# sdu-hpcl/BGSA

Measured on AMD Instinct MI355X. Metric: GCUPS (cell updates/sec) all-pairs Myers 150bp, higher is better.
Workload: dtype u32

## Files before the change

bgsa_amd/__init__.py:

```python
from __future__ import annotations

import ctypes
import os
import subprocess
from pathlib import Path

import numpy as np

HERE = Path(__file__).resolve().parent
LIB_PATH = Path(os.environ["BGSA_HIP_LIB"]) if os.environ.get("BGSA_HIP_LIB") else HERE / "libbgsa_hip.so"
LIB_AB_PATH = HERE / "libbgsa_hip_ab.so"
INCLUDE = HERE.parent / "include" / "bgsa_hip.h"

ALGO_MYERS, ALGO_BANDED, ALGO_BITPAL = 0, 1, 2
DISTANCE_BEYOND = -2
V_NUM = 64

_lib = None


class Params(ctypes.Structure):
    _fields_ = [("algo", ctypes.c_int), ("alignment", ctypes.c_int), ("match", ctypes.c_int),
                ("mismatch", ctypes.c_int), ("gap", ctypes.c_int), ("k", ctypes.c_int)]

# ... 148 lines not shown
    L.bgsa_hip_bucket_release.argtypes = [vp]
    u64p = ctypes.POINTER(ctypes.c_uint64)
    L.bgsa_hip_seam_stats.argtypes = [u64p, u64p, u64p]
    L.bgsa_hip_row_cache_stats.argtypes = [u64p, u64p]
    L.bgsa_hip_event_create.argtypes = [ctypes.POINTER(vp)]
    L.bgsa_hip_event_destroy.argtypes = [vp]
    L.bgsa_hip_event_record.argtypes = [vp, vp]
    L.bgsa_hip_event_synchronize.argtypes = [vp]
    L.bgsa_hip_event_elapsed_ms.argtypes = [vp, vp, ctypes.POINTER(ctypes.c_float)]
    L.bgsa_hip_stream_wait_event.argtypes = [vp, vp]
    L.bgsa_hip_query_stream.argtypes = [i32, vp, i32, i32, vp, i32]
    L.bgsa_hip_myers_band_stream.argtypes = [vp, i32, i32, vp, i32]
    L.bgsa_hip_myers_band_half.argtypes = [i32, i32]
    L.bgsa_hip_myers_band_stats.argtypes = [vp, i32]
    if hasattr(L, "bgsa_hip_myers_band_groups"):
        L.bgsa_hip_myers_band_groups.argtypes = [i32, i64, i32, i32, i32]
    if hasattr(L, "bgsa_hip_myers_band_rescue"):
        L.bgsa_hip_myers_band_rescue.argtypes = [i32, i32, i32, i64]
        L.bgsa_hip_myers_band_rescue_half.argtypes = [i32]
        L.bgsa_hip_myers_band_rescue_stats.argtypes = [vp, i32]
    if hasattr(L, "bgsa_hip_myers_prefix_depths"):
        L.bgsa_hip_myers_prefix_depths.argtypes = [i32, i64, i32, i32, i32, i32, ip, i32]
        L.bgsa_hip_myers_band_segments.argtypes = [vp, i32, i32, ip, i32, vp, i32, ip]
    L.bgsa_hip_kernel_name.argtypes = [i32, i32]
    L.bgsa_hip_kernel_name.restype = ctypes.c_char_p
    L.bgsa_hip_malloc.argtypes = [ctypes.POINTER(vp), sz]
    L.bgsa_hip_free.argtypes = [vp]
    L.bgsa_hip_malloc_host.argtypes = [ctypes.POINTER(vp), sz]
    L.bgsa_hip_free_host.argtypes = [vp]
    L.bgsa_hip_memcpy_h2d.argtypes = [vp, vp, sz, vp]
    L.bgsa_hip_memcpy_d2h.argtypes = [vp, vp, sz, vp]
    L.bgsa_hip_memset.argtypes = [vp, i32, sz, vp]
    L.bgsa_hip_stream_synchronize.argtypes = [vp]
    L.bgsa_hip_stream_create.argtypes = [ctypes.POINTER(vp)]
    L.bgsa_hip_stream_destroy.argtypes = [vp]
    L.bgsa_hip_set_device.argtypes = [i32]
    L.hip_handle_reads.argtypes = [vp, vp, i32, i64, i64]
    L.hip_handle_reads.restype = None
    L.hip_cal_align_score.argtypes = [vp, vp, vp, i32, i32, i32, i32, i32, i32, i32, i32, vp]
    L.hip_cal_align_score.restype = None
    L.align_hip.argtypes = [vp, vp, i32, i32, i32, i32, i32, vp, vp]
    L.align_hip.restype = None
    L.init_mapping_table.restype = None
    L.malloc_mem.argtypes = [ctypes.c_uint64]
    L.malloc_mem.restype = vp
    L.free_mem.argtypes = [vp]
# ... 766 lines not shown
```

bgsa_amd/csrc/bgsa_common.h:

```cpp
#pragma once

#include <hip/hip_runtime.h>
#include <stdint.h>
#include <stdlib.h>
#include <stdio.h>

#include <type_traits>

#include "../../include/bgsa_hip.h"

namespace bgsa {

constexpr int kLanes = HIP_V_NUM;
constexpr int kChars = BGSA_CHAR_NUM;
constexpr int kWavesPerBlock = 4;
constexpr int kMaxWords = 32;

void set_error(const char *what, hipError_t e, const char *file, int line);
void set_error_text(const char *text);
int refuse(const char *who, int rc, const char *why);

#define BGSA_HIP_TRY(expr)                                              \
    do {                                                                \
        hipError_t e_ = (expr);                                         \
// ... 43 lines not shown
    template <typename F>
    static int dispatch(int nw, const char *family, F &&f)
    {
        int rc = BGSA_HIP_EUNSUPPORTED;
        if (((N == nw ? (rc = f(std::integral_constant<int, N>{}), true) : false) || ...)) return rc;
        char msg[128];
        snprintf(msg, sizeof msg, "%s: no kernel of %d words in this build", family, nw);
        set_error_text(msg);
        return BGSA_HIP_EUNSUPPORTED;
    }
    template <int M>
    constexpr Widths<N..., M> with() const { return {}; }
};
template <typename A, typename B> struct JoinWidths;
template <int... A, int... B> struct JoinWidths<Widths<A...>, Widths<B...>> { using type = Widths<A..., B...>; };
template <typename A, typename B> using Join = typename JoinWidths<A, B>::type;

int launch_myers(const ScoreArgs &a, int semi_global = 0);
int launch_myers_place_lens(const ScoreArgs &a);
const char *myers_kernel_name(int word_num, int semi_global = 0);
int myers_band_groups(int word_num, int64_t read_count, int ref_len, int read_len, int mixed_lengths);
int myers_prefix_depths(int word_num, int64_t read_count, int ref_len, int read_len, int n_queries, int mixed_lengths, int *depths);
int myers_band_rescue(int ref_len, int read_len, int n_queries, int64_t read_count);

constexpr int kCodeEnd = 5, kCodeRefill = 6;
inline int stream_windows(int ref_len) { return ref_len / 7 + 1; }
inline size_t stream_stride(int ref_len) { return static_cast<size_t>(stream_windows(ref_len) + 1) * 8; }
__host__ __device__ inline unsigned long long plain_stream_window(const char *row, int ref_len, int i)
{
    const int n_windows = ref_len / 7 + 1;
    unsigned long long win = 0;
    for (int j = 0; j < 8; j++) {
        unsigned code = kCodeEnd;
        if (i < n_windows) {
            const int pos = 7 * i + j;
            if (j == 7) code = (i < n_windows - 1) ? kCodeRefill : kCodeEnd;
            else if (pos < ref_len) {
                code = static_cast<unsigned char>(row[pos]);
                if (code > 4) code = 0;
            }
        }
        win |= static_cast<unsigned long long>(code) << (8 * j);
    }
    return win;
}
int launch_pack_queries(const char *d_content, int ref_len, int ref_start, int ref_end,
// ... 444 lines not shown
```

bgsa_amd/csrc/capi.hip:

```cpp
#include <stdlib.h>
#include <string.h>

#include <algorithm>
#include <atomic>
#include <chrono>
#include <map>
#include <memory>
#include <mutex>
#include <string>
#include <thread>
#include <utility>
#include <vector>

#include "bgsa_common.h"
#include "myers_band.h"

namespace bgsa {

static thread_local std::string g_last_error;

void set_error(const char *what, hipError_t e, const char *file, int line)
{
    char buf[512];
    snprintf(buf, sizeof buf, "%s failed: %s (%s:%d)", what, hipGetErrorString(e), file, line);
// ... 563 lines not shown
    for (int j = 0; j < n && j < cap; j++) depths[j] = d[j];
    return n;
}

int bgsa_hip_myers_band_segments(const char *mapped_row, int ref_len, int read_len, const int *depths, int n_depths,
                                 unsigned char *dst, int cap, int *offsets)
{
    if (!mapped_row || ref_len <= 0 || read_len <= 0 || !depths || n_depths < 1 || n_depths > kPrefixMaxDepths) return 0;
    BandSchedule s;
    if (!band_schedule(ref_len, read_len, band_half(ref_len, read_len), (read_len + 31) / 32, &s)) return 0;
    PrefixPlan p;
    p.n = n_depths;
    for (int j = 0; j < n_depths; j++) p.depth[j] = depths[j];
    if (!prefix_plan_layout(ref_len, (read_len + 31) / 32, s, &p)) return 0;
    const int n = p.off[p.n + 1];
    if (offsets)
        for (int j = 0; j <= p.n + 1; j++) offsets[j] = p.off[j];
    if (dst && cap >= n)
        for (int i = 0; i < n / 8; i++) {
            int seg = 0;
            while (seg < p.n && p.off[seg + 1] <= 8 * i) seg++;
            for (int j = 0; j < 8; j++) dst[8 * i + j] = kCodeEnd;
            band_rows_layout(s, seg ? p.depth[seg - 1] : 0, seg < p.n ? p.depth[seg] : ref_len, seg == p.n, mapped_row, dst + 8 * i,
                             8 * i - p.off[seg], 8);
        }
    return n;
}

int bgsa_hip_myers_band_stream(const char *mapped_row, int ref_len, int read_len, unsigned char *dst, int cap)
{
    if (!mapped_row || ref_len <= 0 || read_len <= 0) return BGSA_HIP_EINVAL;
    BandSchedule s;
    if (!band_schedule(ref_len, read_len, band_half(ref_len, read_len), (read_len + 31) / 32, &s)) return 0;
    const int n = band_stream_layout(ref_len, s, mapped_row, nullptr);
    if (dst && cap >= n)
        for (int i = 0; 8 * i < n; i++) {
            memset(dst + 8 * i, kCodeEnd, 8);
            band_stream_layout(ref_len, s, mapped_row, dst + 8 * i, 8 * i, 8);
        }
    return n;
}

int bgsa_hip_myers_band_stats(unsigned long long *out, int clear)
{
    if (!out) return BGSA_HIP_EINVAL;
    out[0] = out[1] = 0;
// ... 1184 lines not shown
```

bgsa_amd/csrc/myers_band.h:

```cpp
#pragma once

#include <stdlib.h>

#include "bgsa_common.h"

namespace bgsa {

constexpr int kBandMaxWords = 8;
constexpr int kBandMinWords = 3;
constexpr int kBandMaxSwitches = 2 * kBandMaxWords;
constexpr int kCodeSetWin = 7;
constexpr int kBandBadCode = 0xff;

struct BandSchedule {
    int n = 0;
    int row[kBandMaxSwitches] = {};
    int win[kBandMaxSwitches] = {};
};

__host__ __device__ inline int band_window_index(int nw, int a, int b) { return a * nw - a * (a - 1) / 2 + (b - a); }

inline int band_default_half(int len) { return (9 * len + 192) / 32; }

inline int band_rescue_half(int len) { return band_default_half(len) - 3; }

inline int band_half(int m, int n, bool rescue = false)
{
    static const int knob = [] {
        const char *e = getenv("BGSA_MYERS_BAND");
        return e ? atoi(e) : -1;
    }();
    if (knob >= 0) return knob;
    return rescue ? band_rescue_half(m > n ? m : n) : band_default_half(m > n ? m : n);
}

inline bool band_schedule(int m, int n, int h, int nw, BandSchedule *s)
{
    s->n = 0;
    const int B = 2 * h + 1, delta = n - m;
    if (h <= 0 || m <= 0 || n <= 0 || abs(delta) > B || nw < kBandMinWords || nw > kBandMaxWords || (n + 31) / 32 != nw)
        return false;
    const int dlo = -((B - delta) / 2), dhi = (delta + B) / 2;
    long long words = 0;
// ... 1 lines not shown
    for (int i = 1; i <= m; i++) {
        const int jlo = i + dlo < 1 ? 1 : i + dlo, jhi = i + dhi > n ? n : i + dhi;
        const int a = (jlo - 1) / 32, b = (jhi - 1) / 32;
        words += b - a + 1;
        if (a != pa || b != pb) {
            if (s->n == kBandMaxSwitches) {
                s->n = 0;
                return false;
            }
            s->row[s->n] = i - 1;
            s->win[s->n] = band_window_index(nw, a, b);
            s->n++;
            pa = a;
            pb = b;
        }
    }
    if (5 * words > 4ll * m * nw) {
        s->n = 0;
        return false;
    }
    return true;
}

inline size_t band_stream_stride(int ref_len) { return stream_stride(ref_len + 3 * kBandMaxSwitches); }

__host__ __device__ inline int band_rows_layout(const BandSchedule &s, int r0, int r1, bool spare, const char *row, unsigned char *dst,
                                                int first = 0, int count = 0x7fffffff)
{
    int pos = 0, sw = 0;
    auto in = [&]() { return dst && pos >= first && pos - first < count; };
    auto put = [&](int c) {
        if (in()) dst[pos - first] = static_cast<unsigned char>(c);
        pos++;
    };
    auto refill = [&]() {
        put(kCodeRefill);
        while (pos & 7) put(kCodeEnd);
    };
    while (sw + 1 < s.n && s.row[sw + 1] <= r0) sw++;
    for (int r = r0; r < r1; r++) {
        if (dst && pos - first >= count) return pos;
        if (sw < s.n && (s.row[sw] == r || r == r0)) {
            if ((pos & 7) >= 6) refill();
            put(kCodeSetWin);
            put(s.win[sw]);
            sw++;
// ... 122 lines not shown
```

bgsa_amd/csrc/myers_global.hip:

```cpp
#include <stdlib.h>
#include <string.h>

#include <algorithm>

#include "bgsa_common.h"
#include "myers_band.h"

namespace bgsa {

template <int NW, int G, bool SEMI = false>
__device__ __forceinline__ void myers_row(uint32_t (&vp)[G * NW], uint32_t (&vn)[G * NW],
                                          const uint32_t (&eq)[G * NW], int last_word = 0, int last_bit = 0,
                                          int *delta = nullptr)
{
#pragma unroll
  for (int gi = 0; gi < G; gi++) {
    uint32_t hp_prev = 0, hn_prev = 0;
    unsigned carry = 0;
#pragma unroll
    for (int ww = 0; ww < NW; ww++) {
        const int w = gi * NW + ww;
        const uint32_t pv = vp[w], mv = vn[w], e = eq[w];
        const uint32_t pm = e | mv;
        unsigned cout;
// ... 106 lines not shown
    asm volatile("v_mbcnt_lo_u32_b32 %0, -1, 0\n\tv_mbcnt_hi_u32_b32 %0, -1, %0" : "=v"(l));
    return l;
}
constexpr int band_kernel_waves(int nw, int g, bool dyn, bool share)
{
    if (!share) return 1;
    if (g == 2) return nw == 3 ? 8 : (nw == 4 ? (dyn ? 6 : 7) : 5);
    return nw <= 5 ? 8 : (nw == 6 ? (dyn ? 7 : 8) : (nw == 7 ? (dyn ? 6 : 7) : (dyn ? 5 : 6)));
}
template <int NW, int G, bool DYN = false, bool BAND = false, bool LENS = false, bool SHARE = false, bool RESCUE = false>
__global__ __launch_bounds__(256) __attribute__((amdgpu_waves_per_eu(band_kernel_waves(NW, G, DYN, SHARE)))) void myers_global_asm_kernel(
    const unsigned char *__restrict__ streams, const uint32_t *__restrict__ peq,
    int16_t *__restrict__ out, int ref_len, int read_len, long long ld, int n_groups, int word_num,
    int n_queries, int q_tile, int stream_stride_bytes, unsigned *__restrict__ fault_word,
    unsigned *__restrict__ task_counter, int band_limit = 0, unsigned long long *__restrict__ band_launch = nullptr,
    const int32_t *__restrict__ read_lens = nullptr, unsigned long long prefix_segments = 0,
    const PrefixEntry *__restrict__ order = nullptr)
{
    static_assert(!BAND || (NW >= kBandMinWords && NW <= kBandMaxWords && (G == 1 || (G == 2 && NW <= kBandPairMaxWords))),
                  "band: 3..8 words, one subject group per wave — or two up to 5 words");
    static_assert(!(LENS && BAND), "the certified band is derived from one (m, n): a length-aware launch runs full rows");
    static_assert(!SHARE || BAND, "prefix sharing: the band kernels only");
    static_assert(!RESCUE || (BAND && G == 2), "rescue: the two-group band kernels only");
    constexpr bool kLenPerQuery = LENS && NW > 8;
    const int lane = threadIdx.x & (kLanes - 1);
    const unsigned wave_groups = (static_cast<unsigned>(n_groups) + G - 1) / G;
    const unsigned n_tasks = wave_groups * ((static_cast<unsigned>(n_queries) + q_tile - 1) / q_tile);
    unsigned task = 0, task_issued = 0;
    if constexpr (DYN) {
        task = first_wave_task();
        if (task >= n_tasks) return;
    }
    int band_on = 1, unreported = 0;
    [[maybe_unused]] auto reporting_lane = [&]() {
        if constexpr (RESCUE) {
            return lane_now() == 0;
        } else
            return lane == 0;
    };
    do {
        int group0, tile;
        if constexpr (DYN) {
            group0 = static_cast<int>((task % wave_groups) * G);
            tile = static_cast<int>(task / wave_groups);
        } else {
            group0 = __builtin_amdgcn_readfirstlane((blockIdx.x * kWavesPerBlock + (threadIdx.x >> 6)) * G);
// ... 27 lines not shown
        for (int k = q0; k < q1; k++) {
            if constexpr (DYN) {
                if (k == q1 - 1) task_issued = issue_wave_task(task_counter);
            }
            int q = k, seg = 0;
            if constexpr (SHARE) {
                const int2 e = *reinterpret_cast<const int2 *>(order + k);
                q = __builtin_amdgcn_readfirstlane(e.x);
                seg = __builtin_amdgcn_readfirstlane(e.y >> 16);
            }
            uint32_t st[2 * G * NW];
#pragma unroll
            for (int w = 0; w < G * NW; w++) {
                st[2 * w] = ~0u;
                st[2 * w + 1] = 0u;
            }
            const unsigned long long s =
                reinterpret_cast<unsigned long long>(streams) + static_cast<unsigned long long>(q) * stream_stride_bytes;
            if constexpr (BAND) {
                const int n_live = G == 1 ? 1 : (group0 + 1 < n_groups ? 2 : 1);
                const int tried = band_on * n_live;
                int band = band_on, score[G];
                const int n_depths = SHARE ? static_cast<int>(prefix_segments >> 56) : 0;
                const bool sharing = SHARE && band_on;
                [[maybe_unused]] auto wave_slots = [&]() {
                    if constexpr (RESCUE) {
                        return prefix_slots + __builtin_amdgcn_readfirstlane((threadIdx.x >> 6) * G) * kLanes + lane_now();
                    } else
                        return prefix_slots + ((threadIdx.x >> 6) * G) * kLanes + lane;
                };
                if (!sharing) seg = 0;
                if (SHARE && seg) {
                    const uint4 *const slots = wave_slots();
#pragma unroll
                    for (int gi = 0; gi < G; gi++) {
                        const uint4 v = slots[((seg - 1) * kWavesPerBlock * G + gi) * kLanes];
                        st[2 * gi * NW] = v.x;
                        st[2 * gi * NW + 1] = v.y;
                        st[2 * gi * NW + 2] = v.z;
                        st[2 * gi * NW + 3] = v.w;
                    }
                }
                for (;;) {
                    for (; seg <= n_depths; seg++) {
                        const int at = SHARE ? static_cast<int>((prefix_segments >> (8 * seg)) & 0xffu) * 8 : 0;
                        const int left = myers_band_rows_asm<NW, G>(st, P, uniform_u64(s + static_cast<unsigned>(at)),
                                                                    __builtin_amdgcn_readfirstlane((stream_stride_bytes - at) / 8 - 2),
                                                                    __builtin_amdgcn_readfirstlane(band));
                        note_stream_fault(fault_word, left);
                        if (SHARE && sharing && band && seg < n_depths) {
                            uint4 *const slots = wave_slots();
#pragma unroll
                            for (int gi = 0; gi < G; gi++)
                                slots[(seg * kWavesPerBlock * G + gi) * kLanes] =
                                    make_uint4(st[2 * gi * NW], st[2 * gi * NW + 1], st[2 * gi * NW + 2], st[2 * gi * NW + 3]);
                        }
                    }
#pragma unroll
                    for (int gi = 0; gi < G; gi++) {
                        score[gi] = ref_len;
#pragma unroll
                        for (int w = 0; w < NW; w++) {
                            const int rem = read_len - 32 * w;
                            const uint32_t m = rem >= 32 ? ~0u : (rem <= 0 ? 0u : ((1u << rem) - 1u));
                            score[gi] += __popc(st[2 * (gi * NW + w)] & m) - __popc(st[2 * (gi * NW + w) + 1] & m);
                        }
                    }
                    if (!band) break;
                    int n_over = 0;
#pragma unroll
                    for (int gi = 0; gi < G; gi++)
                        if (gi < n_live && __builtin_amdgcn_ballot_w64(score[gi] > band_limit) != 0) n_over++;
                    if (n_over == 0) break;
                    if constexpr (G == 1) n_over = 1;
                    if constexpr (RESCUE) {
                        const unsigned c0 = __popcll(__builtin_amdgcn_ballot_w64(score[0] > band_limit)),
                                       c1 = n_live > 1 ? __popcll(__builtin_amdgcn_ballot_w64(score[1] > band_limit)) : 0u;
                        unsigned forced = (c0 > kRescueMaxLanes ? 1u : 0u) + (c1 > kRescueMaxLanes ? 1u : 0u);
                        if (forced == 0) {
                            unsigned *const words = reinterpret_cast<unsigned *>(band_launch) - 16;
                            unsigned long long claim = 0;
                            if (reporting_lane()) claim = atomicAdd(rescue_claimed(words), static_cast<unsigned long long>(c0 + c1));
                            const unsigned base = __builtin_amdgcn_readfirstlane(static_cast<unsigned>(claim)),
                                           base_hi = __builtin_amdgcn_readfirstlane(static_cast<unsigned>(claim >> 32));
                            const unsigned capacity = __builtin_amdgcn_readfirstlane(*rescue_capacity(words));
                            const unsigned room = (base_hi == 0 && base < capacity) ? capacity - base : 0u;
                            const bool fits = c0 + c1 <= room;
                            RescueEntry *const mine = rescue_pool(words) + base;
                            const unsigned column = lane_now() + static_cast<unsigned>(group0) * kLanes;
#pragma unroll
                            for (int gi = 0; gi < G; gi++) {
                                const bool up = gi < n_live && score[gi] > band_limit;
                                const unsigned long long over = __builtin_amdgcn_ballot_w64(up);
                                const unsigned at = (gi ? c0 : 0u) + __builtin_amdgcn_mbcnt_hi(static_cast<unsigned>(over >> 32),
                                                                                              __builtin_amdgcn_mbcnt_lo(static_cast<unsigned>(over), 0u));
                                if (up && at < room)
                                    mine[at] = fits ? RescueEntry{q, static_cast<int>(column + gi * kLanes)} : RescueEntry{-1, -1};
                            }
                            if (fits) break;
                            forced = static_cast<unsigned>(n_over);
                        }
                        if (reporting_lane()) atomicAdd(&band_launch[3], static_cast<unsigned long long>(forced));
                    }
                    band = 0;
                    seg = 0;
                    unsigned long long r = static_cast<unsigned long long>(n_over),
                                       b = static_cast<unsigned long long>(unreported) + n_live;
                    if (reporting_lane()) {
                        r += atomicAdd(&band_launch[0], r);
                        b += atomicAdd(&band_launch[1], b);
                    }
                    r = uniform_u64(r);
                    b = uniform_u64(b);
                    unreported = -n_live;
                    if (b >= 64 && 8 * r > b) band_on = 0;
#pragma unroll
                    for (int w = 0; w < G * NW; w++) {
                        st[2 * w] = ~0u;
                        st[2 * w + 1] = 0u;
                    }
                }
                unreported += tried;
#pragma unroll
                for (int gi = 0; gi < G; gi++)
                    if (gi < n_live && !(RESCUE && band && score[gi] > band_limit))
                        dst[static_cast<size_t>(q) * ld + gi * kLanes] = static_cast<int16_t>(-score[gi]);
            } else {
                int left;
                if constexpr (NW <= kPairMaxWords)
                    left = myers_pair_rows_asm<NW, G>(st, P, uniform_u64(s), __builtin_amdgcn_readfirstlane(stream_stride_bytes / 8 - 2));
                else
                    left = myers_rows_asm<NW, G>(st, P, uniform_u64(s), __builtin_amdgcn_readfirstlane(stream_stride_bytes / 8 - 2));
                note_stream_fault(fault_word, left);
#pragma unroll
                for (int gi = 0; gi < G; gi++) {
                    int score = ref_len;
                    int n_cols = read_len;
                    if constexpr (kLenPerQuery) {
                        const unsigned lane_e = lane_now();
                        n_cols = group0 + gi < n_groups ? lane_read_len(read_lens, static_cast<size_t>(group0 + gi) * kLanes + lane_e, read_len) : 0;
                    }
                    else if constexpr (LENS)
                        n_cols = own_len[gi];
                    if constexpr (LENS) asm volatile("" : "+v"(n_cols));
#pragma unroll
                    for (int w = 0; w < NW; w++) {
                        const int rem = n_cols - 32 * w;
                        const uint32_t m = rem >= 32 ? ~0u : (rem <= 0 ? 0u : ((1u << rem) - 1u));
// ... 483 lines not shown
long long rescue_entries_for(int ref_len, int read_len, int nq, int64_t read_count)
{
    if (read_len < kRescueMinLen || read_len > kRescueMaxLen || nq <= 0 || read_count < 2 * kLanes || read_count > 0x7fffffffll) return 0;
    const long long pool = static_cast<long long>(rescue_pool_bytes(read_len, nq) / sizeof(RescueEntry));
    long long entries = rescue_pool_entries(read_len, nq);
    if (rescue_pool_knob() >= 0 && rescue_pool_knob() < entries) entries = rescue_pool_knob();
    if (rescue_knob() >= 0) return rescue_knob() ? entries : 0;
    if (!kRescueDefault || nq < kRescueMinQueries || read_count < kBandPairMinReads || !band_rescue_lengths(ref_len, read_len)) return 0;
    return 2e-3 * nq * static_cast<double>(read_count) <= static_cast<double>(pool / 2) ? entries : 0;
}
int band_half_for(int ref_len, int read_len, int nw, int groups, int nq, int64_t read_count, BandSchedule *sched, long long *entries)
{
    *entries = groups == 2 && nw <= kBandPairMaxWords ? rescue_entries_for(ref_len, read_len, nq, read_count) : 0;
    if (*entries > 0) {
        const int h = band_half(ref_len, read_len, true);
        if (band_schedule(ref_len, read_len, h, nw, sched)) return h;
        *entries = 0;
    }
    const int h = band_half(ref_len, read_len);
    band_schedule(ref_len, read_len, h, nw, sched);
    return h;
}

template <int NW>
__global__ __launch_bounds__(256) void myers_band_rescue_kernel(unsigned *__restrict__ words, const char *__restrict__ content,
                                                                const uint32_t *__restrict__ peq, int16_t *__restrict__ out,
                                                                int ref_len, int read_len, long long ld, int word_num, int ref_start,
                                                                int n_queries)
{
    const unsigned long long claimed = *rescue_claimed(words), capacity = *rescue_capacity(words);
    const unsigned long long count = claimed < capacity ? claimed : capacity;
    const RescueEntry *pool = rescue_pool(words);
    const unsigned lane = threadIdx.x & (kLanes - 1);
    const unsigned long long n_waves = static_cast<unsigned long long>(gridDim.x) * kWavesPerBlock;
    unsigned rescued = 0;
    for (unsigned long long chunk = static_cast<unsigned long long>(blockIdx.x) * kWavesPerBlock + (threadIdx.x >> 6);
         chunk * kLanes < count; chunk += n_waves) {
        const unsigned long long at = chunk * kLanes + lane;
        RescueEntry e = pool[at < count ? at : count - 1];
        const bool live = at < count && e.q >= 0 && e.q < n_queries && e.subject >= 0 && e.subject < ld;
        if (!live) e = RescueEntry{0, 0};
        const uint32_t *g = peq + (static_cast<size_t>(e.subject / kLanes) * kChars * word_num) * kLanes + e.subject % kLanes;
        uint32_t P[kChars][NW], pv[NW], mv[NW];
#pragma unroll
        for (int c = 0; c < kChars; c++)
#pragma unroll
// ... 41 lines not shown
    const bool lens = a.d_read_lens != nullptr;
    const int64_t n_waves = (a.n_groups() + G - 1) / G;
    const TaskPlan plan = plan_tasks(nq, n_waves, static_cast<long long>(a.ref_len) * NW * G, NW >= 30 ? 8 : 32, kCounter,
                                     NW >= 30 ? long_query_tile() : query_tile_max(), lens);
    if (lens && kCounter && !plan.dynamic) {
        set_error_text("myers: too many tasks for one length-aware launch (split the query window)");
        return BGSA_HIP_EUNSUPPORTED;
    }
    note_query_tile(plan.q_tile);
    AsmKernel on_grid = nullptr, on_counter = nullptr;
    if constexpr (!kBandPair) {
        on_grid = myers_global_asm_kernel<NW, G, false>;
        if constexpr (kCounter) on_counter = myers_global_asm_kernel<NW, G, true>;
        if (lens) {
            if constexpr (kCounter) on_grid = nullptr, on_counter = myers_global_asm_kernel<NW, G, true, false, true>;
            else on_grid = myers_global_asm_kernel<NW, G, false, false, true>;
        }
    }
    BandSchedule sched;
    PrefixPlan prefix;
    int h = 0;
    bool band = false;
    long long rescue = 0;
    if constexpr ((G == 1 || kBandPair) && NW >= kBandMinWords && NW <= kBandMaxWords) {
        if (!lens) h = band_half_for(a.ref_len, a.read_len, NW, G, nq, a.read_count, &sched, &rescue);
        band = !lens && sched.n > 0;
        if (band) {
            on_grid = myers_global_asm_kernel<NW, G, false, true>;
            on_counter = myers_global_asm_kernel<NW, G, true, true>;
            prefix_select(a.ref_len, NW, sched, nq, plan.q_tile, a.read_count, &prefix);
            if (prefix.n) {
                on_grid = myers_global_asm_kernel<NW, G, false, true, false, true>;
                on_counter = myers_global_asm_kernel<NW, G, true, true, false, true>;
            }
            if constexpr (kBandPair) {
                if (rescue > 0) {
                    on_grid = prefix.n ? myers_global_asm_kernel<NW, G, false, true, false, true, true>
                                       : myers_global_asm_kernel<NW, G, false, true, false, false, true>;
                    on_counter = prefix.n ? myers_global_asm_kernel<NW, G, true, true, false, true, true>
                                          : myers_global_asm_kernel<NW, G, true, true, false, false, true>;
                }
            }
        }
    }
    if (kBandPair && !band) {
        set_error_text("myers: two subject groups per wave selected for a launch without the certified band");
        return BGSA_HIP_EUNSUPPORTED;
    }
    const unsigned lds = (plan.dynamic ? myers_lds_pad() : 0u) + static_cast<unsigned>(prefix_lds_bytes(prefix, G));
    const int stride = static_cast<int>(prefix.n  ? static_cast<size_t>(prefix.off[prefix.n + 1])
                                        : band    ? band_stream_stride(a.ref_len)
                                        : kPairs  ? pair_stream_stride(a.ref_len)
                                                  : stream_stride(a.ref_len));
    unsigned *words = task_counter_in(a.d_workspace, static_cast<size_t>(stride) * nq);
    LaunchGrid lg;
    if (int rc = plan_grid(plan, n_waves, nq, words,
                           [&] { return on_counter ? persistent_blocks_for(on_counter, lds) : persistent_blocks(); }, "myers", &lg))
        return rc;
    if (prefix.n)
        if (int rc = launch_prefix_order(a.d_content, a.ref_len, a.ref_start, a.ref_end, plan.q_tile, prefix, words, a.stream))
            return rc;
    if (int rc = prefix.n ? launch_pack_band_segments(a.d_content, a.ref_len, sched, prefix, a.ref_start, a.ref_end, a.d_workspace, a.stream, words,
                                                       static_cast<unsigned>(rescue))
                 : band   ? launch_pack_band(a.d_content, a.ref_len, sched, a.ref_start, a.ref_end, a.d_workspace, a.stream, words,
                                             static_cast<unsigned>(rescue))
                 : kPairs ? launch_pack_query_pairs(a.d_content, a.ref_len, a.ref_start, a.ref_end, a.d_workspace, a.stream, lg.counter)
                          : launch_pack_queries(a.d_content, a.ref_len, a.ref_start, a.ref_end, a.d_workspace, a.stream, lg.counter))
        return rc;
    unsigned *fault = nullptr;
    if (int rc = stream_guard(a.d_workspace, stride, kPairs ? kPairRefill : kCodeRefill, band ? kBandBadCode : kPairs ? -1 : 7, a.stream, &fault))
        return rc;
    unsigned long long *guard = band ? band_launch_words(words) : nullptr;
    const AsmKernel kernel = lg.counter ? on_counter : on_grid;
    hipLaunchKernelGGL(kernel, lg.grid, dim3(256), lds, a.stream,
                       static_cast<const unsigned char *>(a.d_workspace), a.d_peq, a.results<int16_t>(), a.ref_len, a.read_len,
                       static_cast<long long>(a.read_count), static_cast<int>(a.n_groups()), a.word_num, nq, plan.q_tile, stride,
                       fault, lg.counter, band ? 2 * h + 1 : 0, guard, a.d_read_lens, prefix_segments_word(prefix),
                       static_cast<const PrefixEntry *>(prefix_entries(words)));
    BGSA_HIP_TRY(hipGetLastError());
    if constexpr (kBandPair) {
        if (rescue > 0) {
            hipLaunchKernelGGL(myers_band_rescue_kernel<NW>, dim3(persistent_blocks()), dim3(256), 0, a.stream, words, a.d_content, a.d_peq,
                               a.results<int16_t>(), a.ref_len, a.read_len, static_cast<long long>(a.read_count), a.word_num,
                               a.ref_start, nq);
            BGSA_HIP_TRY(hipGetLastError());
        }
    }
    if (band) {
        hipLaunchKernelGGL(band_stats_add_kernel, dim3(1), dim3(1), 0, a.stream, static_cast<const unsigned long long *>(guard),
                           band_stats_words(fault));
        BGSA_HIP_TRY(hipGetLastError());
    }
    return BGSA_HIP_OK;
}

template <int NW, bool LENS = false>
int launch_semi_asm(const ScoreArgs &a)
{
    const int nq = a.nq(), stride = static_cast<int>(stream_stride(a.ref_len));
    const int q_tile = pick_q_tile(nq, a.n_groups(), a.ref_len, NW);
// ... 181 lines not shown

int myers_band_groups(int word_num, int64_t read_count, int ref_len, int read_len, int mixed_lengths)
{
    if (word_num < 1 || word_num > kMaxWords) return 1;
    const MyersChoice c = myers_select(word_num, 0, read_count, ref_len, read_len, mixed_lengths != 0);
    return c.family == MyersFamily::kAsmBandPairs ? 2 : 1;
}

int myers_prefix_depths(int word_num, int64_t read_count, int ref_len, int read_len, int n_queries, int mixed_lengths, int *depths)
{
    if (word_num < 1 || word_num > kMaxWords || n_queries < 1) return 0;
    const MyersChoice c = myers_select(word_num, 0, read_count, ref_len, read_len, mixed_lengths != 0);
    if ((c.family != MyersFamily::kAsm && c.family != MyersFamily::kAsmBandPairs) || mixed_lengths) return 0;
    BandSchedule sched;
    long long rescue = 0;
    band_half_for(ref_len, read_len, c.nw, c.G, n_queries, read_count, &sched, &rescue);
    if (sched.n == 0) return 0;
    const int64_t n_waves = (read_count / kLanes + c.G - 1) / c.G;
    const TaskPlan plan = plan_tasks(n_queries, n_waves, static_cast<long long>(ref_len) * c.nw * c.G, 32, true, query_tile_max());
    PrefixPlan p;
    prefix_select(ref_len, c.nw, sched, n_queries, plan.q_tile, read_count, &p);
    for (int j = 0; j < p.n; j++) depths[j] = p.depth[j];
    return p.n;
}

int myers_band_rescue(int ref_len, int read_len, int n_queries, int64_t read_count)
{
    if (ref_len <= 0 || read_len <= 0 || n_queries < 1 || read_count < 1) return 0;
    const int word_num = (read_len + 31) / 32;
    if (word_num > kMaxWords) return 0;
    const MyersChoice c = myers_select(word_num, 0, read_count, ref_len, read_len, false);
    if (c.family != MyersFamily::kAsmBandPairs) return 0;
    BandSchedule sched;
    long long rescue = 0;
    const int h = band_half_for(ref_len, read_len, c.nw, c.G, n_queries, read_count, &sched, &rescue);
    return rescue > 0 ? h : 0;
}

const char *myers_kernel_name(int word_num, int semi_global)
{
    static thread_local char name[64];
    const MyersChoice c = myers_select(word_num, semi_global, 2 * kLanes);
    switch (c.family) {
    case MyersFamily::kAsm:
    case MyersFamily::kAsmBandPairs:
    case MyersFamily::kAsmPairs: snprintf(name, sizeof name, "myers_global_asm_kernel<%d, %d>", c.nw, c.G); break;
// ... 76 lines not shown
```

bgsa_amd/csrc/rows_ir.py:

```python
#!/usr/bin/env python3
from __future__ import annotations

import functools
import os
from dataclasses import dataclass, field

import numpy as np


def _knob(name: str, default: str) -> str:
    return os.environ.get(f"BGSA_GEN_{name}", default)


CLASS_CODE = np.zeros(256, dtype=np.uint8)
CLASS_CODE[list(b"ACGTN")] = range(5)


def class_code(ch) -> int:
    return int(CLASS_CODE[int(ch)])


def _low_mask(bits: int) -> np.uint32:
    return np.uint32(0xFFFFFFFF if bits >= 32 else (0 if bits <= 0 else (1 << bits) - 1))

# ... 536 lines not shown
                return f"S{int(x[1:]) + 2 * (g * nw + a)}"
            if x.startswith("E"):
                return f"E{int(x[1:]) + g * nw + a}"
            if g and x and not x.startswith("$"):
                return f"{x[0]}{g}{x[2:]}"
            return x

        out.ops += [Op(op.kind, ren(op.dst), tuple(ren(s) for s in op.srcs), op.imm, op.dst2) for op in src.ops]
    return out


def myers_window_index(nw: int, a: int, b: int) -> int:
    return a * nw - a * (a - 1) // 2 + (b - a)


def myers_band_half(length: int) -> int:
    return (9 * length + 192) // 32


def myers_band_rescue_half(length: int) -> int:
    return myers_band_half(length) - 3


def myers_band_windows(m: int, n: int, h: int, nw: int):
    B = 2 * h + 1
    delta = n - m
    if h <= 0 or abs(delta) > B or nw > MYERS_BAND_MAX_WORDS or nw < 3:
        return None
    dlo, dhi = -((B - delta) // 2), (delta + B) // 2
    out = []
    for i in range(1, m + 1):
        jlo, jhi = max(1, i + dlo), min(n, i + dhi)
        out.append(((jlo - 1) // 32, (jhi - 1) // 32))
    if 5 * sum(b - a + 1 for a, b in out) > 4 * m * nw:
        return None
    return out


def myers_band_stream(codes, m: int, n: int, h: int, nw: int) -> bytes | None:
    win = myers_band_windows(m, n, h, nw)
    if win is None:
        return None
    out = bytearray()

    def refill():
        out.append(6)
        while len(out) % 8:
            out.append(5)

    def put(c):
        if len(out) % 8 == 7:
            refill()
        out.append(c)

    cur = None
    for i in range(m):
        if win[i] != cur:
            if len(out) % 8 >= 6:
                refill()
            out += bytes([7, myers_window_index(nw, *win[i])])
            cur = win[i]
        put(int(codes[i]))
    put(5)
    while len(out) % 8:
        out.append(5)
    out += bytes([5] * 8)
    return bytes(out)


def myers_band_segments(codes, m: int, n: int, h: int, nw: int, depths) -> tuple[bytes, list] | None:
    win = myers_band_windows(m, n, h, nw)
    depths = list(depths)
    if win is None or not depths or depths != sorted(set(depths)) or depths[0] < 1 or depths[-1] >= m:
        return None
    if any(w not in ((0, 0), (0, 1)) for w in win[:depths[-1]]):
        return None
    out, offsets = bytearray(), []
    cuts = [0] + depths + [m]
    for j in range(len(cuts) - 1):
        offsets.append(len(out))
        seg = bytearray()
        cur = None
        for i in range(cuts[j], cuts[j + 1]):
            if win[i] != cur:
                if len(seg) % 8 >= 6:
                    seg += bytes([6] + [5] * (7 - len(seg) % 8))
                seg += bytes([7, myers_window_index(nw, *win[i])])
                cur = win[i]
            if len(seg) % 8 == 7:
                seg.append(6)
            seg.append(int(codes[i]))
        if len(seg) % 8 == 7:
            seg.append(6)
        seg.append(5)
# ... 12 lines not shown
    cur = (0, nw - 1)
    pos, rows = 0, 0
    while True:
        c = stream[pos]
        if c == 5:
            return rows
        if c == 6:
            pos = (pos | 7) + 1
            continue
        if c == 7:
            k = stream[pos + 1]
            assert k < len(windows) and myers_window_index(nw, *windows[k]) == k
            cur = windows[k] if band else (0, nw - 1)
            pos += 2
            continue
        assert c < 5
        if cur not in bodies:
            bodies[cur] = myers_window_body(nw, *cur, groups=groups, balanced=balanced)
            if schedule is not None:
                bodies[cur] = schedule(bodies[cur])
        bodies[cur].simulate(state, [peq[c, w] for w in range(groups * nw)], cls=c)
        rows += cur[1] - cur[0] + 1
        pos += 1


def myers_body10(nw: int, groups: int = 1) -> Body:
    b = Body()
    for g in range(groups):
        _myers_ten(b, nw, *_state(g * nw), lambda w: f"E{g * nw + w}", f"d{g}_{{w}}", f"hp{g}_{{w}}", f"hn{g}_{{w}}")
    return b


def myers_semi_body(nw: int, split: int = 0) -> Body:
    return _myers_semi_rows(nw, lambda b: (lambda w: f"E{w}"), "hn{w}", split)


def _myers_semi_rows(nw: int, mask, hn: str | None, split: int = 0) -> Body:
    b = Body()
    RUN, BEST = f"S{2 * nw}", f"S{2 * nw + 1}"
    less, more = (lambda: b.SUBBZ(RUN)), (lambda: b.ADDCZ(RUN))
    if MYERS_EIGHT:
        _myers_eight(b, nw, *_state(), mask(b), split=split, edge=0, tap=(less, more), place={"take1": "m2"})
    else:
        _myers_ten(b, nw, *_state(), mask(b), hn=hn, edge=0, tap=(more, less), early=2)
    b.MINU(BEST, BEST, RUN)
    return b
# ... 971 lines not shown
```

include/bgsa_hip.h:

```cpp
#ifndef BGSA_HIP_H
#define BGSA_HIP_H

#include <stddef.h>
#include <stdint.h>

#ifdef __cplusplus
extern "C" {
#endif

#define BGSA_CHAR_NUM 5
#define HIP_V_NUM 64
#define HIP_WORD_SIZE 32
#define HIP_BANDED_WORD_SIZE 64
#define HIP_MAX_ERROR 127
typedef uint32_t hip_read_t;
typedef uint32_t hip_data_t;
typedef int16_t hip_write_t;
typedef int8_t hip_banded_write_t;

#ifndef BGSA_HAVE_SEQ_T
#define BGSA_HAVE_SEQ_T
typedef struct _seq_t {
    int len;
    int64_t size;
// ... 274 lines not shown
    const int32_t *d_read_len, *d_strand;
    const int64_t *d_ref_begin, *d_ref_end;
    const int32_t *d_distance, *d_n_ops, *d_flag, *d_mapq, *d_rnext;
    const int64_t *d_pnext, *d_tlen;
} bgsa_hip_sam_batch_t;
int bgsa_hip_sam_mapq_dev(const int32_t *d_scores, const int32_t *d_keep, int64_t ns, int k, int bound, int32_t *d_primary, int32_t *d_mapq,
                          int32_t *d_n1, int32_t *d_d2, void *stream);
int bgsa_hip_sam_measure_dev(const bgsa_hip_sam_batch_t *batch, int64_t n, int64_t *d_lengths, int32_t *d_malformed, void *stream);
int bgsa_hip_sam_emit_dev(const bgsa_hip_sam_batch_t *batch, int64_t n, const int64_t *d_offsets, uint8_t *d_text, int64_t text_bytes,
                          int32_t *d_malformed, void *stream);

#define BGSA_HIP_FAULT_BUDGET 1
#define BGSA_HIP_FAULT_CODE 2
#define BGSA_HIP_FAULT_PAIR 4
#define BGSA_HIP_FAULT_BAND 8
int bgsa_hip_stream_faults(int clear);
int bgsa_hip_debug_inject_stream_fault(int kind);

int bgsa_hip_clock_probe_start(int n_probes, unsigned max_ms, void *caller_stream);
int bgsa_hip_clock_probe_stop(double *mhz, int *xcc, int cap, int *n_out, double *seconds);

int bgsa_hip_query_stream(int algo, const char *mapped_row, int ref_len, int k, unsigned char *dst, int cap);

int bgsa_hip_myers_band_rescue_half(int len);
int bgsa_hip_myers_band_rescue(int ref_len, int read_len, int n_queries, int64_t read_count);
int bgsa_hip_myers_band_rescue_stats(unsigned long long *out, int clear);
int bgsa_hip_myers_prefix_depths(int word_num, int64_t read_count, int ref_len, int read_len, int n_queries, int mixed_lengths,
                                 int *depths, int cap);
int bgsa_hip_myers_band_segments(const char *mapped_row, int ref_len, int read_len, const int *depths, int n_depths,
                                 unsigned char *dst, int cap, int *offsets);
int bgsa_hip_myers_band_stream(const char *mapped_row, int ref_len, int read_len, unsigned char *dst, int cap);
int bgsa_hip_myers_band_half(int ref_len, int read_len);
int bgsa_hip_myers_band_groups(int word_num, int64_t read_count, int ref_len, int read_len, int mixed_lengths);
int bgsa_hip_myers_band_stats(unsigned long long *out, int clear);

int bgsa_hip_last_query_tile(void);

const char *bgsa_hip_kernel_name(int algo, int word_num);

#ifdef __cplusplus
}
#endif
#endif
```

Measured before the change: 406,300.

## Prune low band words after certified cut rows in Myers rescue band kernel

Adds per-length tables of early cut points (row, word) for the two-group rescue band path. After each cut row, the band schedule drops the lower 32-bit words, so fewer words are processed per row. To stay certified, the kernel computes a tighter per-lane limit from the partial score at each cut word and sends lanes over that limit to rescue. This cuts band work at the cost of more lanes possibly needing rescue, plus extra popcount and compare logic in the epilogue.

```diff
diff --git a/bgsa_amd/__init__.py b/bgsa_amd/__init__.py
--- a/bgsa_amd/__init__.py
+++ b/bgsa_amd/__init__.py
@@ -194,6 +194,10 @@
     if hasattr(L, "bgsa_hip_myers_prefix_depths"):
         L.bgsa_hip_myers_prefix_depths.argtypes = [i32, i64, i32, i32, i32, i32, ip, i32]
         L.bgsa_hip_myers_band_segments.argtypes = [vp, i32, i32, ip, i32, vp, i32, ip]
+    if hasattr(L, "bgsa_hip_myers_band_early"):
+        L.bgsa_hip_myers_band_early.argtypes = [i32, i32, i32, i64, ip]
+        L.bgsa_hip_myers_band_early_cuts.argtypes = [i32, i32, ip, ip]
+        L.bgsa_hip_myers_band_early_segments.argtypes = [vp, i32, i32, ip, ip, i32, ip, i32, vp, i32, ip]
     L.bgsa_hip_kernel_name.argtypes = [i32, i32]
     L.bgsa_hip_kernel_name.restype = ctypes.c_char_p
     L.bgsa_hip_malloc.argtypes = [ctypes.POINTER(vp), sz]
diff --git a/bgsa_amd/csrc/bgsa_common.h b/bgsa_amd/csrc/bgsa_common.h
--- a/bgsa_amd/csrc/bgsa_common.h
+++ b/bgsa_amd/csrc/bgsa_common.h
@@ -89,6 +89,7 @@
 int myers_band_groups(int word_num, int64_t read_count, int ref_len, int read_len, int mixed_lengths);
 int myers_prefix_depths(int word_num, int64_t read_count, int ref_len, int read_len, int n_queries, int mixed_lengths, int *depths);
 int myers_band_rescue(int ref_len, int read_len, int n_queries, int64_t read_count);
+int myers_band_early(int ref_len, int read_len, int n_queries, int64_t read_count, int *rows, int *words);
 
 constexpr int kCodeEnd = 5, kCodeRefill = 6;
 inline int stream_windows(int ref_len) { return ref_len / 7 + 1; }
diff --git a/bgsa_amd/csrc/capi.hip b/bgsa_amd/csrc/capi.hip
--- a/bgsa_amd/csrc/capi.hip
+++ b/bgsa_amd/csrc/capi.hip
@@ -609,6 +609,60 @@
             while (seg < p.n && p.off[seg + 1] <= 8 * i) seg++;
             for (int j = 0; j < 8; j++) dst[8 * i + j] = kCodeEnd;
             band_rows_layout(s, seg ? p.depth[seg - 1] : 0, seg < p.n ? p.depth[seg] : ref_len, seg == p.n, mapped_row, dst + 8 * i,
+                             8 * i - p.off[seg], 8);
+        }
+    return n;
+}
+
+int bgsa_hip_myers_band_early(int ref_len, int read_len, int n_queries, int64_t read_count, int *rows_out)
+{
+    return myers_band_early(ref_len, read_len, n_queries, read_count, rows_out, nullptr);
+}
+
+int bgsa_hip_myers_band_early_cuts(int len, int h, int *rows, int *words)
+{
+    if (len <= 0) return 0;
+    const BandCuts c = band_early_cuts(len, len, h);
+    for (int j = 0; j < c.n; j++) {
+        if (rows) rows[j] = c.row[j];
+        if (words) words[j] = c.word[j];
+    }
+    return c.n;
+}
+
+int bgsa_hip_myers_band_early_segments(const char *mapped_row, int len, int h, const int *cut_rows, const int *cut_words, int n_cuts,
+                                       const int *depths, int n_depths, unsigned char *dst, int cap, int *offsets)
+{
+    if (!mapped_row || len <= 0 || n_cuts < 1 || n_cuts > kBandMaxCuts || !cut_rows || !cut_words || n_depths < 0 ||
+        (n_depths && !depths) || n_depths > kPrefixMaxDepths)
+        return 0;
+    BandCuts c;
+    c.n = n_cuts;
+    for (int j = 0; j < n_cuts; j++) c.row[j] = cut_rows[j], c.word[j] = cut_words[j];
+    BandSchedule s;
+    if (!band_schedule_early(len, len, h, (len + 31) / 32, c, &s)) return 0;
+    if (n_depths == 0) {
+        const int n = band_stream_layout(len, s, mapped_row, nullptr);
+        if (offsets) offsets[0] = 0, offsets[1] = n;
+        if (dst && cap >= n)
+            for (int i = 0; 8 * i < n; i++) {
+                memset(dst + 8 * i, kCodeEnd, 8);
+                band_stream_layout(len, s, mapped_row, dst + 8 * i, 8 * i, 8);
+            }
+        return n;
+    }
+    PrefixPlan p;
+    for (int j = 0; j < n_depths; j++) p.depth[p.n++] = depths[j];
+    if (!prefix_plan_layout(len, (len + 31) / 32, s, &p)) return 0;
+    const int n = p.off[p.n + 1];
+    if (offsets)
+        for (int j = 0; j <= p.n + 1; j++) offsets[j] = p.off[j];
+    if (dst && cap >= n)
+        for (int i = 0; i < n / 8; i++) {
+            int seg = 0;
+            while (seg < p.n && p.off[seg + 1] <= 8 * i) seg++;
+            for (int j = 0; j < 8; j++) dst[8 * i + j] = kCodeEnd;
+            band_rows_layout(s, seg ? p.depth[seg - 1] : 0, seg < p.n ? p.depth[seg] : len, seg == p.n, mapped_row, dst + 8 * i,
                              8 * i - p.off[seg], 8);
         }
     return n;
diff --git a/bgsa_amd/csrc/myers_band.h b/bgsa_amd/csrc/myers_band.h
--- a/bgsa_amd/csrc/myers_band.h
+++ b/bgsa_amd/csrc/myers_band.h
@@ -19,6 +19,12 @@
 };
 
 __host__ __device__ inline int band_window_index(int nw, int a, int b) { return a * nw - a * (a - 1) / 2 + (b - a); }
+inline void band_window_of(int nw, int win, int *a, int *b)
+{
+    *a = 0;
+    while (*a + 1 < nw && band_window_index(nw, *a + 1, *a + 1) <= win) ++*a;
+    *b = *a + win - band_window_index(nw, *a, *a);
+}
 
 inline int band_default_half(int len) { return (9 * len + 192) / 32; }
 
@@ -66,6 +72,98 @@
     return true;
 }
 
+constexpr int kBandMaxCuts = 2;
+struct BandCuts {
+    int n = 0;
+    int row[kBandMaxCuts] = {};
+    int word[kBandMaxCuts] = {};
+};
+struct BandEarlyEntry {
+    int len, n, row[kBandMaxCuts], word[kBandMaxCuts];
+};
+constexpr BandEarlyEntry kBandEarlyCuts[] = {
+    {68, 1, {51, 0}, {0, 0}},
+    {96, 2, {60, 83}, {0, 1}},
+    {100, 2, {62, 85}, {0, 1}},
+    {107, 2, {64, 88}, {0, 1}},
+    {111, 2, {65, 89}, {0, 1}},
+    {114, 2, {66, 90}, {0, 1}},
+    {118, 2, {67, 92}, {0, 1}},
+    {121, 2, {68, 93}, {0, 1}},
+    {125, 2, {69, 94}, {0, 1}},
+    {128, 2, {70, 95}, {0, 1}},
+    {132, 2, {71, 96}, {0, 1}},
+    {139, 2, {99, 121}, {1, 2}},
+    {143, 2, {100, 122}, {1, 2}},
+    {146, 2, {101, 123}, {1, 2}},
+    {150, 2, {106, 130}, {1, 2}},
+    {153, 2, {104, 126}, {1, 2}},
+    {157, 2, {105, 128}, {1, 2}},
+    {160, 2, {106, 129}, {1, 2}},
+};
+inline BandCuts band_early_cuts(int m, int n, int h)
+{
+    BandCuts c;
+    if (m != n || h != band_rescue_half(n)) return c;
+    for (const BandEarlyEntry &e : kBandEarlyCuts)
+        if (e.len == n) {
+            c.n = e.n;
+            for (int j = 0; j < e.n; j++) c.row[j] = e.row[j], c.word[j] = e.word[j];
+        }
+    return c;
+}
+constexpr int kBandEarlyLimitBits = 10, kBandEarlyCutBits = 11;
+constexpr int kBandEarlyLimitMask = (1 << kBandEarlyLimitBits) - 1;
+inline int band_early_word(int band_limit, const BandCuts &c)
+{
+    unsigned v = static_cast<unsigned>(band_limit) & kBandEarlyLimitMask;
+    for (int j = 0; j < c.n; j++)
+        v |= (static_cast<unsigned>(2 * c.row[j] - 32 * (c.word[j] + 1)) | static_cast<unsigned>(c.word[j]) << 9)
+             << (kBandEarlyLimitBits + kBandEarlyCutBits * j);
+    return static_cast<int>(v);
+}
+inline bool band_schedule_early(int m, int n, int h, int nw, const BandCuts &cuts, BandSchedule *s)
+{
+    if (cuts.n == 0) return band_schedule(m, n, h, nw, s);
+    BandSchedule base;
+    s->n = 0;
+    if (m != n || cuts.n < 0 || cuts.n > kBandMaxCuts || !band_schedule(m, n, h, nw, &base)) return false;
+    for (int j = 0; j < cuts.n; j++)
+        if (cuts.word[j] < 0 || cuts.word[j] >= nw - 1 || cuts.row[j] < 32 * (cuts.word[j] + 1) || cuts.row[j] >= m ||
+            (j && (cuts.row[j] <= cuts.row[j - 1] || cuts.word[j] <= cuts.word[j - 1])))
+            return false;
+    int pw = -1, sw = 0;
+    for (int r = 0; r < m; r++) {
+        while (sw + 1 < base.n && base.row[sw + 1] <= r) sw++;
+        int a, b;
+        band_window_of(nw, base.win[sw], &a, &b);
+        for (int j = 0; j < cuts.n; j++)
+            if (r >= cuts.row[j] && a < cuts.word[j] + 1) a = cuts.word[j] + 1;
+        if (a > b || s->n == kBandMaxSwitches) {
+            s->n = 0;
+            return false;
+        }
+        const int win = band_window_index(nw, a, b);
+        if (win != pw) {
+            s->row[s->n] = r;
+            s->win[s->n] = win;
+            s->n++;
+            pw = win;
+        }
+    }
+    return true;
+}
+inline long long band_schedule_word_rows(int m, int nw, const BandSchedule &s)
+{
+    long long words = 0;
+    for (int i = 0; i < s.n; i++) {
+        int a, b;
+        band_window_of(nw, s.win[i], &a, &b);
+        words += static_cast<long long>((i + 1 < s.n ? s.row[i + 1] : m) - s.row[i]) * (b - a + 1);
+    }
+    return words;
+}
+
 inline size_t band_stream_stride(int ref_len) { return stream_stride(ref_len + 3 * kBandMaxSwitches); }
 
 __host__ __device__ inline int band_rows_layout(const BandSchedule &s, int r0, int r1, bool spare, const char *row, unsigned char *dst,
diff --git a/bgsa_amd/csrc/myers_global.hip b/bgsa_amd/csrc/myers_global.hip
--- a/bgsa_amd/csrc/myers_global.hip
+++ b/bgsa_amd/csrc/myers_global.hip
@@ -152,6 +152,7 @@
     static_assert(!(LENS && BAND), "the certified band is derived from one (m, n): a length-aware launch runs full rows");
     static_assert(!SHARE || BAND, "prefix sharing: the band kernels only");
     static_assert(!RESCUE || (BAND && G == 2), "rescue: the two-group band kernels only");
+    constexpr bool kEarly = RESCUE;
     constexpr bool kLenPerQuery = LENS && NW > 8;
     const int lane = threadIdx.x & (kLanes - 1);
     const unsigned wave_groups = (static_cast<unsigned>(n_groups) + G - 1) / G;
@@ -225,6 +226,8 @@
                 const int tried = band_on * n_live;
                 int band = band_on, score[G];
                 const int n_depths = SHARE ? static_cast<int>(prefix_segments >> 56) : 0;
+                [[maybe_unused]] unsigned long long over[G];
+                [[maybe_unused]] auto is_over = [&](int gi) { return ((over[gi] >> lane_now()) & 1ull) != 0; };
                 const bool sharing = SHARE && band_on;
                 [[maybe_unused]] auto wave_slots = [&]() {
                     if constexpr (RESCUE) {
@@ -259,26 +262,52 @@
                                     make_uint4(st[2 * gi * NW], st[2 * gi * NW + 1], st[2 * gi * NW + 2], st[2 * gi * NW + 3]);
                         }
                     }
-#pragma unroll
-                    for (int gi = 0; gi < G; gi++) {
-                        score[gi] = ref_len;
-#pragma unroll
-                        for (int w = 0; w < NW; w++) {
-                            const int rem = read_len - 32 * w;
-                            const uint32_t m = rem >= 32 ? ~0u : (rem <= 0 ? 0u : ((1u << rem) - 1u));
-                            score[gi] += __popc(st[2 * (gi * NW + w)] & m) - __popc(st[2 * (gi * NW + w) + 1] & m);
+                    if constexpr (kEarly) {
+                        unsigned packed = static_cast<unsigned>(band_limit);
+                        asm volatile("" : "+s"(packed));
+                        int cut_word[kBandMaxCuts], cut_add[kBandMaxCuts];
+#pragma unroll
+                        for (int j = 0; j < kBandMaxCuts; j++) {
+                            const unsigned cut = (packed >> (kBandEarlyLimitBits + kBandEarlyCutBits * j)) & ((1u << kBandEarlyCutBits) - 1u);
+                            cut_word[j] = cut ? static_cast<int>(cut >> 9) : -1;
+                            cut_add[j] = static_cast<int>(cut & 0x1ffu) - ref_len;
+                        }
+#pragma unroll
+                        for (int gi = 0; gi < G; gi++) {
+                            score[gi] = ref_len;
+                            int limit = static_cast<int>(packed & kBandEarlyLimitMask);
+#pragma unroll
+                            for (int w = 0; w < NW; w++) {
+                                const int rem = read_len - 32 * w;
+                                const uint32_t m = rem >= 32 ? ~0u : (rem <= 0 ? 0u : ((1u << rem) - 1u));
+                                score[gi] += __popc(st[2 * (gi * NW + w)] & m) - __popc(st[2 * (gi * NW + w) + 1] & m);
+#pragma unroll
+                                for (int j = 0; j < kBandMaxCuts; j++)
+                                    if (w < NW - 1 && w == cut_word[j]) limit = score[gi] + cut_add[j] < limit ? score[gi] + cut_add[j] : limit;
+                            }
+                            over[gi] = __builtin_amdgcn_ballot_w64(score[gi] > limit);
+                        }
+                    } else {
+#pragma unroll
+                        for (int gi = 0; gi < G; gi++) {
+                            score[gi] = ref_len;
+#pragma unroll
+                            for (int w = 0; w < NW; w++) {
+                                const int rem = read_len - 32 * w;
+                                const uint32_t m = rem >= 32 ? ~0u : (rem <= 0 ? 0u : ((1u << rem) - 1u));
+                                score[gi] += __popc(st[2 * (gi * NW + w)] & m) - __popc(st[2 * (gi * NW + w) + 1] & m);
+                            }
                         }
                     }
                     if (!band) break;
                     int n_over = 0;
 #pragma unroll
                     for (int gi = 0; gi < G; gi++)
-                        if (gi < n_live && __builtin_amdgcn_ballot_w64(score[gi] > band_limit) != 0) n_over++;
+                        if (gi < n_live && (kEarly ? over[gi] : __builtin_amdgcn_ballot_w64(score[gi] > band_limit)) != 0) n_over++;
                     if (n_over == 0) break;
                     if constexpr (G == 1) n_over = 1;
                     if constexpr (RESCUE) {
-                        const unsigned c0 = __popcll(__builtin_amdgcn_ballot_w64(score[0] > band_limit)),
-                                       c1 = n_live > 1 ? __popcll(__builtin_amdgcn_ballot_w64(score[1] > band_limit)) : 0u;
+                        const unsigned c0 = __popcll(over[0]), c1 = n_live > 1 ? __popcll(over[1]) : 0u;
                         unsigned forced = (c0 > kRescueMaxLanes ? 1u : 0u) + (c1 > kRescueMaxLanes ? 1u : 0u);
                         if (forced == 0) {
                             unsigned *const words = reinterpret_cast<unsigned *>(band_launch) - 16;
@@ -293,7 +322,7 @@
                             const unsigned column = lane_now() + static_cast<unsigned>(group0) * kLanes;
 #pragma unroll
                             for (int gi = 0; gi < G; gi++) {
-                                const bool up = gi < n_live && score[gi] > band_limit;
+                                const bool up = gi < n_live && is_over(gi);
                                 const unsigned long long over = __builtin_amdgcn_ballot_w64(up);
                                 const unsigned at = (gi ? c0 : 0u) + __builtin_amdgcn_mbcnt_hi(static_cast<unsigned>(over >> 32),
                                                                                               __builtin_amdgcn_mbcnt_lo(static_cast<unsigned>(over), 0u));
@@ -326,7 +355,7 @@
                 unreported += tried;
 #pragma unroll
                 for (int gi = 0; gi < G; gi++)
-                    if (gi < n_live && !(RESCUE && band && score[gi] > band_limit))
+                    if (gi < n_live && !(RESCUE && band && is_over(gi)))
                         dst[static_cast<size_t>(q) * ld + gi * kLanes] = static_cast<int16_t>(-score[gi]);
             } else {
                 int left;
@@ -856,6 +885,26 @@
     return h;
 }
 
+constexpr bool kEarlyDefault = true;
+static int early_knob()
+{
+    static const int v = [] {
+        const char *e = getenv("BGSA_MYERS_BAND_EARLY");
+        return (e && (e[0] == '0' || e[0] == '1') && e[1] == 0) ? e[0] - '0' : -1;
+    }();
+    return v;
+}
+BandCuts early_select(int ref_len, int read_len, int nw, int h, long long rescue, BandSchedule *sched)
+{
+    if (rescue <= 0 || early_knob() == 0) return BandCuts{};
+    if (early_knob() < 0 && (!kEarlyDefault || rescue_knob() >= 0)) return BandCuts{};
+    const BandCuts cuts = band_early_cuts(ref_len, read_len, h);
+    BandSchedule early;
+    if (cuts.n == 0 || !band_schedule_early(ref_len, read_len, h, nw, cuts, &early)) return BandCuts{};
+    *sched = early;
+    return cuts;
+}
+
 template <int NW>
 __global__ __launch_bounds__(256) void myers_band_rescue_kernel(unsigned *__restrict__ words, const char *__restrict__ content,
                                                                 const uint32_t *__restrict__ peq, int16_t *__restrict__ out,
@@ -943,12 +992,14 @@
     int h = 0;
     bool band = false;
     long long rescue = 0;
+    BandCuts cuts;
     if constexpr ((G == 1 || kBandPair) && NW >= kBandMinWords && NW <= kBandMaxWords) {
         if (!lens) h = band_half_for(a.ref_len, a.read_len, NW, G, nq, a.read_count, &sched, &rescue);
         band = !lens && sched.n > 0;
         if (band) {
             on_grid = myers_global_asm_kernel<NW, G, false, true>;
             on_counter = myers_global_asm_kernel<NW, G, true, true>;
+            if constexpr (kBandPair) cuts = early_select(a.ref_len, a.read_len, NW, h, rescue, &sched);
             prefix_select(a.ref_len, NW, sched, nq, plan.q_tile, a.read_count, &prefix);
             if (prefix.n) {
                 on_grid = myers_global_asm_kernel<NW, G, false, true, false, true>;
@@ -963,6 +1014,10 @@
                 }
             }
         }
+    }
+    if (band && 2 * h + 1 > kBandEarlyLimitMask) {
+        set_error_text("myers band: half-width out of range");
+        return BGSA_HIP_EINVAL;
     }
     if (kBandPair && !band) {
         set_error_text("myers: two subject groups per wave selected for a launch without the certified band");
@@ -996,7 +1051,7 @@
     hipLaunchKernelGGL(kernel, lg.grid, dim3(256), lds, a.stream,
                        static_cast<const unsigned char *>(a.d_workspace), a.d_peq, a.results<int16_t>(), a.ref_len, a.read_len,
                        static_cast<long long>(a.read_count), static_cast<int>(a.n_groups()), a.word_num, nq, plan.q_tile, stride,
-                       fault, lg.counter, band ? 2 * h + 1 : 0, guard, a.d_read_lens, prefix_segments_word(prefix),
+                       fault, lg.counter, band ? band_early_word(2 * h + 1, cuts) : 0, guard, a.d_read_lens, prefix_segments_word(prefix),
                        static_cast<const PrefixEntry *>(prefix_entries(words)));
     BGSA_HIP_TRY(hipGetLastError());
     if constexpr (kBandPair) {
@@ -1224,6 +1279,25 @@
     prefix_select(ref_len, c.nw, sched, n_queries, plan.q_tile, read_count, &p);
     for (int j = 0; j < p.n; j++) depths[j] = p.depth[j];
     return p.n;
+}
+
+int myers_band_early(int ref_len, int read_len, int n_queries, int64_t read_count, int *rows, int *words)
+{
+    if (ref_len <= 0 || read_len <= 0 || n_queries < 1 || read_count < 1) return 0;
+    const int word_num = (read_len + 31) / 32;
+    if (word_num > kMaxWords) return 0;
+    const MyersChoice c = myers_select(word_num, 0, read_count, ref_len, read_len, false);
+    if (c.family != MyersFamily::kAsmBandPairs) return 0;
+    BandSchedule sched;
+    long long rescue = 0;
+    const int h = band_half_for(ref_len, read_len, c.nw, c.G, n_queries, read_count, &sched, &rescue);
+    if (sched.n == 0) return 0;
+    const BandCuts cuts = early_select(ref_len, read_len, c.nw, h, rescue, &sched);
+    for (int j = 0; j < cuts.n; j++) {
+        if (rows) rows[j] = cuts.row[j];
+        if (words) words[j] = cuts.word[j];
+    }
+    return cuts.n;
 }
 
 int myers_band_rescue(int ref_len, int read_len, int n_queries, int64_t read_count)
diff --git a/bgsa_amd/csrc/rows_ir.py b/bgsa_amd/csrc/rows_ir.py
--- a/bgsa_amd/csrc/rows_ir.py
+++ b/bgsa_amd/csrc/rows_ir.py
@@ -582,7 +582,41 @@
     return myers_band_half(length) - 3
 
 
-def myers_band_windows(m: int, n: int, h: int, nw: int):
+MYERS_BAND_EARLY_CUTS = {
+    68: ((51, 0),),
+    96: ((60, 0), (83, 1)),
+    100: ((62, 0), (85, 1)),
+    107: ((64, 0), (88, 1)),
+    111: ((65, 0), (89, 1)),
+    114: ((66, 0), (90, 1)),
+    118: ((67, 0), (92, 1)),
+    121: ((68, 0), (93, 1)),
+    125: ((69, 0), (94, 1)),
+    128: ((70, 0), (95, 1)),
+    132: ((71, 0), (96, 1)),
+    139: ((99, 1), (121, 2)),
+    143: ((100, 1), (122, 2)),
+    146: ((101, 1), (123, 2)),
+    150: ((106, 1), (130, 2)),
+    153: ((104, 1), (126, 2)),
+    157: ((105, 1), (128, 2)),
+    160: ((106, 1), (129, 2)),
+}
+
+
+def myers_band_early_cuts(length: int, h: int):
+    return MYERS_BAND_EARLY_CUTS.get(length, ()) if h == myers_band_rescue_half(length) else ()
+
+
+def myers_band_windows(m: int, n: int, h: int, nw: int, cuts=()):
+    if cuts:
+        base = myers_band_windows(m, n, h, nw)
+        cuts = list(cuts)
+        if base is None or m != n or len(cuts) > 2 or any(not (0 <= w < nw - 1 and 32 * (w + 1) <= r < m) for r, w in cuts) or \
+                any(x[0] >= y[0] or x[1] >= y[1] for x, y in zip(cuts, cuts[1:])):
+            return None
+        out = [(max([a] + [w + 1 for r, w in cuts if i > r]), b) for i, (a, b) in enumerate(base, start=1)]
+        return None if any(a > b for a, b in out) else out
     B = 2 * h + 1
     delta = n - m
     if h <= 0 or abs(delta) > B or nw > MYERS_BAND_MAX_WORDS or nw < 3:
@@ -597,8 +631,8 @@
     return out
 
 
-def myers_band_stream(codes, m: int, n: int, h: int, nw: int) -> bytes | None:
-    win = myers_band_windows(m, n, h, nw)
+def myers_band_stream(codes, m: int, n: int, h: int, nw: int, cuts=()) -> bytes | None:
+    win = myers_band_windows(m, n, h, nw, cuts) if cuts else myers_band_windows(m, n, h, nw)
     if win is None:
         return None
     out = bytearray()
@@ -628,8 +662,8 @@
     return bytes(out)
 
 
-def myers_band_segments(codes, m: int, n: int, h: int, nw: int, depths) -> tuple[bytes, list] | None:
-    win = myers_band_windows(m, n, h, nw)
+def myers_band_segments(codes, m: int, n: int, h: int, nw: int, depths, cuts=()) -> tuple[bytes, list] | None:
+    win = myers_band_windows(m, n, h, nw, cuts) if cuts else myers_band_windows(m, n, h, nw)
     depths = list(depths)
     if win is None or not depths or depths != sorted(set(depths)) or depths[0] < 1 or depths[-1] >= m:
         return None
@@ -688,6 +722,17 @@
         bodies[cur].simulate(state, [peq[c, w] for w in range(groups * nw)], cls=c)
         rows += cur[1] - cur[0] + 1
         pos += 1
+
+
+def run_band_early(nw: int, peq: np.ndarray, codes, m: int, h: int, cuts, groups: int = 1, **kw):
+    lanes = peq.shape[2]
+    state = myers_init_state(nw, groups, lanes)
+    rows = run_band_stream(nw, state, peq, myers_band_stream(codes, m, m, h, nw, cuts), groups=groups, **kw)
+    limit = [np.full(lanes, 2 * h + 1, dtype=np.int64) for _ in range(groups)]
+    for r, w in cuts:
+        for g in range(groups):
+            limit[g] = np.minimum(limit[g], 2 * r - 32 * (w + 1) + _myers_columns(state[2 * g * nw:], w + 1, 32 * (w + 1)))
+    return [m + _myers_columns(state[2 * g * nw:], nw, m) for g in range(groups)], limit, rows
 
 
 def myers_body10(nw: int, groups: int = 1) -> Body:
diff --git a/include/bgsa_hip.h b/include/bgsa_hip.h
--- a/include/bgsa_hip.h
+++ b/include/bgsa_hip.h
@@ -320,6 +320,10 @@
 
 int bgsa_hip_query_stream(int algo, const char *mapped_row, int ref_len, int k, unsigned char *dst, int cap);
 
+int bgsa_hip_myers_band_early(int ref_len, int read_len, int n_queries, int64_t read_count, int *rows_out);
+int bgsa_hip_myers_band_early_cuts(int len, int h, int *rows, int *words);
+int bgsa_hip_myers_band_early_segments(const char *mapped_row, int len, int h, const int *cut_rows, const int *cut_words, int n_cuts,
+                                       const int *depths, int n_depths, unsigned char *dst, int cap, int *offsets);
 int bgsa_hip_myers_band_rescue_half(int len);
 int bgsa_hip_myers_band_rescue(int ref_len, int read_len, int n_queries, int64_t read_count);
 int bgsa_hip_myers_band_rescue_stats(unsigned long long *out, int clear);
```

Result: faster. 411,500, median of 6 (+1.3%).
